# databricks/spark-deep-learning

Measured on AMD Instinct MI355X. Metric: images/sec, higher is better.
Workload: dtype bf16; 1 GPU; model=resnet50, global_batch=512, image=224, parallelism=dp1

## Files before the change

sparkdl/models/resnet.py:

```python

import torch
import torch.nn as nn

from sparkdl.ops import BatchNormAct2d, Conv1x1, batch_norm_relu_maxpool


class Bottleneck(nn.Module):
    expansion = 4

    def __init__(self, cin, width, stride=1):
        super().__init__()
        cout = width * self.expansion
        self.conv1 = Conv1x1(cin, width)
        self.bn1 = BatchNormAct2d(width, relu=True)
        self.conv2 = nn.Conv2d(width, width, 3, stride=stride, padding=1,
                               bias=False)
        self.bn2 = BatchNormAct2d(width, relu=True)
        self.conv3 = Conv1x1(width, cout)
        self.bn3 = BatchNormAct2d(cout, relu=True)
        if stride != 1 or cin != cout:
            self.down_conv = Conv1x1(cin, cout, stride=stride)
            self.down_bn = BatchNormAct2d(cout, relu=False)
        else:
            self.down_conv = None

    def forward(self, x):
        if self.down_conv is not None:
            idn = self.down_bn(self.down_conv(x))
        else:
            idn = x
        out = self.bn1(self.conv1(x))
        out = self.bn2(self.conv2(out))
        return self.bn3(self.conv3(out), residual=idn)


class ResNet50(nn.Module):
    LAYERS = (3, 4, 6, 3)

    def __init__(self, num_classes=1000):
        super().__init__()
        self.stem_conv = nn.Conv2d(3, 64, 7, stride=2, padding=3,
                                   bias=False)
        self.stem_bn = BatchNormAct2d(64, relu=True)
        self.stem_pool = nn.MaxPool2d(3, stride=2, padding=1)
        cin = 64
        stages = []
        for i, blocks in enumerate(self.LAYERS):
            width = 64 * (2 ** i)
            stride = 1 if i == 0 else 2
            layer = []
            for b in range(blocks):
                layer.append(Bottleneck(cin, width, stride if b == 0 else 1))
                cin = width * Bottleneck.expansion
            stages.append(nn.Sequential(*layer))
        self.stages = nn.Sequential(*stages)
        self.pool = nn.AdaptiveAvgPool2d(1)
        self.fc = nn.Linear(2048, num_classes)

        for m in self.modules():
            if isinstance(m, nn.Conv2d):
                nn.init.kaiming_normal_(m.weight, mode="fan_out",
                                        nonlinearity="relu")
        for m in self.modules():
            if isinstance(m, Bottleneck):
                nn.init.zeros_(m.bn3.weight)

    def forward(self, x):
        bn = self.stem_bn
        x = batch_norm_relu_maxpool(
            self.stem_conv(x), bn.weight, bn.bias, bn.running_mean,
            bn.running_var, momentum=bn.momentum, eps=bn.eps,
            training=bn.training)
        x = self.stages(x)
        x = self.pool(x).flatten(1)
        return self.fc(x)
```

sparkdl/ops/csrc/batchnorm.hip:

```cpp

#include "common.hip.h"
#include "kernels.h"

namespace {

constexpr int kBlock = 256;
constexpr int kVec = 8;
constexpr int kUnroll = 2;
constexpr int kFoldFloats = kBlock * 2 * kVec;
constexpr int kFinCh = 4;

__device__ __forceinline__ float bn_affine(short x, float scale,
                                           float shift) {
  return bf2f(x) * scale + shift;
}
__device__ __forceinline__ float bn_xhat(short x, float mean, float rstd) {
  return (bf2f(x) - mean) * rstd;
}
__device__ __forceinline__ float bn_dx(float d, float xh, float k1,
                                       float k2, float k3) {
  return k1 * (d - k2 - xh * k3);
}


// ... 247 lines not shown
      if (RELU) mbits = mask[base / kVec];
      accum(xv, dv, mbits);
    }
  }
  bn_block_fold(lds, s1, s2, rpb, row_off, lane_col, cols,
                slab + (size_t)blockIdx.x * 2 * cols);
}

__global__ __launch_bounds__(kBlock) void bn_bwd_finalize_k(
    const float* __restrict__ slab, int G, const float* __restrict__ gamma,
    const float* __restrict__ save_rstd, float* __restrict__ dgamma,
    float* __restrict__ dbeta, float* __restrict__ c1,
    float* __restrict__ c2, float* __restrict__ c3, long long rows,
    int cols, int training) {
  __shared__ float red[kBlock / WAVE * 2 * kFinCh];
  float sum_dym, sum_dymxh;
  const int blk = bn_fin_block();
  bn_slab_sum(slab, G, cols, blk, red, sum_dym, sum_dymxh);
  if (threadIdx.x >= kFinCh) return;
  const int c = blk * kFinCh + threadIdx.x;
  dgamma[c] = sum_dymxh;
  dbeta[c] = sum_dym;
  c1[c] = gamma[c] * save_rstd[c];
  if (training) {
    c2[c] = sum_dym / rows;
    c3[c] = sum_dymxh / rows;
  } else {
    c2[c] = 0.f;
    c3[c] = 0.f;
  }
}

template <bool RELU, bool RES>
__global__ __launch_bounds__(kBlock) void bn_bwd_apply_k(
    const short* __restrict__ x, const unsigned char* __restrict__ mask,
    const short* __restrict__ dy, const float* __restrict__ save_mean,
    const float* __restrict__ save_rstd, const float* __restrict__ c1,
    const float* __restrict__ c2, const float* __restrict__ c3,
    short* __restrict__ dx, short* __restrict__ dres, long long rows,
    int cols) {
  const int tpr = cols / kVec;
  const int rpb = kBlock / min(tpr, kBlock);
  const int lane_col = (threadIdx.x % tpr) * kVec;
  const int row_off = threadIdx.x / tpr;
  if (row_off >= rpb) return;
  const float4v m0 = *(const float4v*)(save_mean + lane_col);
  const float4v m1 = *(const float4v*)(save_mean + lane_col + 4);
  const float4v r0 = *(const float4v*)(save_rstd + lane_col);
  const float4v r1 = *(const float4v*)(save_rstd + lane_col + 4);
  const float4v a0 = *(const float4v*)(c1 + lane_col);
  const float4v a1 = *(const float4v*)(c1 + lane_col + 4);
  const float4v b0 = *(const float4v*)(c2 + lane_col);
  const float4v b1 = *(const float4v*)(c2 + lane_col + 4);
  const float4v g0 = *(const float4v*)(c3 + lane_col);
  const float4v g1 = *(const float4v*)(c3 + lane_col + 4);

  for (long long r = (long long)blockIdx.x * rpb + row_off; r < rows;
       r += (long long)gridDim.x * rpb) {
    const long long base = r * cols + lane_col;
    const short8 xv = *(const short8*)(x + base);
    const short8 dv = *(const short8*)(dy + base);
    unsigned char mbits = 0xffu;
    if (RELU) mbits = mask[base / kVec];
    short8 odx, odr;
#pragma unroll
    for (int j = 0; j < kVec; ++j) {
      float d = bf2f(dv[j]);
      if (RELU && !(mbits & (1u << j))) d = 0.f;
      const float mean = j < 4 ? m0[j] : m1[j - 4];
      const float rstd = j < 4 ? r0[j] : r1[j - 4];
      const float xh = bn_xhat(xv[j], mean, rstd);
      const float k1 = j < 4 ? a0[j] : a1[j - 4];
      const float k2 = j < 4 ? b0[j] : b1[j - 4];
      const float k3 = j < 4 ? g0[j] : g1[j - 4];
      odx[j] = f2bf(bn_dx(d, xh, k1, k2, k3));
      if (RES) odr[j] = f2bf(d);
    }
    *(short8*)(dx + base) = odx;
    if (RES) *(short8*)(dres + base) = odr;
  }
}


typedef unsigned uint2v __attribute__((ext_vector_type(2)));

constexpr unsigned kPoolDead = 9;
constexpr unsigned kPoolNone = 0xffu;

struct PoolGeom {
  int H, W, Ho, Wo;
};

__global__ __launch_bounds__(kBlock) void bn_apply_pool_k(
    const short* __restrict__ x, const float* __restrict__ scale,
    const float* __restrict__ shift, short* __restrict__ pooled,
    unsigned char* __restrict__ code, long long orows, int cols,
    PoolGeom g) {
  const int tpr = cols / kVec;
  const int rpb = kBlock / min(tpr, kBlock);
  const int lane_col = (threadIdx.x % tpr) * kVec;
  const int row_off = threadIdx.x / tpr;
  if (row_off >= rpb) return;
  const float4v sc0 = *(const float4v*)(scale + lane_col);
  const float4v sc1 = *(const float4v*)(scale + lane_col + 4);
  const float4v sh0 = *(const float4v*)(shift + lane_col);
  const float4v sh1 = *(const float4v*)(shift + lane_col + 4);
  const unsigned opix = (unsigned)(g.Ho * g.Wo);

  for (long long o = (long long)blockIdx.x * rpb + row_off; o < orows;
       o += (long long)gridDim.x * rpb) {
    const unsigned n = (unsigned)o / opix;
    const unsigned rem = (unsigned)o - n * opix;
    const int oh = (int)(rem / (unsigned)g.Wo);
    const int ow = (int)(rem - (unsigned)oh * (unsigned)g.Wo);
    short8 v[9];
#pragma unroll
    for (int kh = 0; kh < 3; ++kh) {
      const int ih = min(max(2 * oh - 1 + kh, 0), g.H - 1);
#pragma unroll
      for (int kw = 0; kw < 3; ++kw) {
        const int iw = min(max(2 * ow - 1 + kw, 0), g.W - 1);
        const long long r = ((long long)n * g.H + ih) * g.W + iw;
        v[kh * 3 + kw] = *(const short8*)(x + r * cols + lane_col);
      }
    }
    float best[kVec], bestf[kVec];
    unsigned tap[kVec];
#pragma unroll
    for (int j = 0; j < kVec; ++j) {
      best[j] = -INFINITY;
      bestf[j] = 0.f;
      tap[j] = 0;
    }
#pragma unroll
    for (int kh = 0; kh < 3; ++kh) {
      const int ih = 2 * oh - 1 + kh;
      const bool hin = ih >= 0 && ih < g.H;
#pragma unroll
      for (int kw = 0; kw < 3; ++kw) {
        const int iw = 2 * ow - 1 + kw;
        const bool in = hin && iw >= 0 && iw < g.W;
#pragma unroll
        for (int j = 0; j < kVec; ++j) {
          const float f =
              bn_affine(v[kh * 3 + kw][j], j < 4 ? sc0[j] : sc1[j - 4],
                        j < 4 ? sh0[j] : sh1[j - 4]);
          const float q = bf2f(f2bf(fmaxf(f, 0.f)));
          if (in && q > best[j]) {
            best[j] = q;
            bestf[j] = f;
            tap[j] = kh * 3 + kw;
          }
        }
      }
    }
    short8 ov;
    unsigned c0 = 0, c1 = 0;
#pragma unroll
    for (int j = 0; j < kVec; ++j) {
      union { float f; unsigned u; } b;
      b.f = best[j];
      ov[j] = (short)(b.u >> 16);
      const unsigned c = bestf[j] > 0.f ? tap[j] : kPoolDead;
      if (j < 4) c0 |= c << (8 * j);
      else c1 |= c << (8 * (j - 4));
    }
// ... 147 lines not shown
      const float rstd = j < 4 ? r0[j] : r1[j - 4];
      const float xh = bn_xhat(xv[j], mean, rstd);
      const float k1 = j < 4 ? a0[j] : a1[j - 4];
      const float k2 = j < 4 ? b0[j] : b1[j - 4];
      const float k3 = j < 4 ? g0[j] : g1[j - 4];
      odx[j] = f2bf(bn_dx(d[j], xh, k1, k2, k3));
    }
    *(short8*)(dx + base) = odx;
  }
}

int bn_grid(long long rows, int cols) {
  const int tpr = cols / kVec;
  const int rpb = kBlock / min(tpr, kBlock);
  long long blocks = (rows + rpb - 1) / rpb;
  return (int)min(blocks, 2048LL);
}

}

int bn_reduce_blocks(long long rows, int cols) {
  const int tpr = cols / kVec;
  const int rpb = kBlock / min(tpr, kBlock);
  const long long row_blocks = (rows + rpb - 1) / rpb;
  const long long g = max(256LL, min(512LL, rows / 64));
  return (int)max(1LL, min(row_blocks, g));
}

long long bn_scratch_floats(long long rows, int cols) {
  return (long long)bn_reduce_blocks(rows, cols) * 2 * cols + 3LL * cols;
}

void launch_bn_fwd(const short* x, const short* res, const float* gamma,
                   const float* beta, float* running_mean,
                   float* running_var, float* save_mean, float* save_rstd,
                   float* scratch, short* y, unsigned char* mask,
                   long long rows, int cols, float momentum, float eps,
                   bool training, bool relu, hipStream_t stream) {
  const int grid = bn_grid(rows, cols);
  const int G = bn_reduce_blocks(rows, cols);
  if (training)
    hipLaunchKernelGGL(bn_stats_k<kUnroll>, dim3(G), dim3(kBlock), 0,
                       stream, x, scratch, rows, cols);
  float* scale = scratch + (size_t)G * 2 * cols;
  float* shift = scale + cols;
  hipLaunchKernelGGL(bn_finalize_k, dim3(cols / kFinCh), dim3(kBlock), 0,
                     stream, scratch, G, gamma, beta, running_mean,
                     running_var, save_mean, save_rstd, scale, shift, rows,
                     cols, momentum, eps, (int)training);
  auto ap = relu ? (res ? bn_apply_k<true, true> : bn_apply_k<true, false>)
                 : (res ? bn_apply_k<false, true>
                        : bn_apply_k<false, false>);
  hipLaunchKernelGGL(ap, dim3(grid), dim3(kBlock), 0, stream, x, res,
                     scale, shift, y, mask, rows, cols);
}

void launch_bn_bwd(const short* x, const unsigned char* mask,
                   const short* dy, const float* gamma,
                   const float* save_mean, const float* save_rstd,
                   float* scratch, float* dgamma, float* dbeta, short* dx,
                   short* dres, long long rows, int cols, bool training,
                   bool relu, hipStream_t stream) {
  const int grid = bn_grid(rows, cols);
  const int G = bn_reduce_blocks(rows, cols);
  auto rk = relu ? bn_bwd_reduce_k<true, kUnroll>
                 : bn_bwd_reduce_k<false, kUnroll>;
  hipLaunchKernelGGL(rk, dim3(G), dim3(kBlock), 0, stream, x, mask, dy,
                     save_mean, save_rstd, scratch, rows, cols);
  float* c1 = scratch + (size_t)G * 2 * cols;
  float* c2 = c1 + cols;
  float* c3 = c2 + cols;
  hipLaunchKernelGGL(bn_bwd_finalize_k, dim3(cols / kFinCh), dim3(kBlock),
                     0, stream, scratch, G, gamma, save_rstd, dgamma, dbeta,
                     c1, c2, c3, rows, cols, (int)training);
  auto ak = relu ? (dres ? bn_bwd_apply_k<true, true>
                         : bn_bwd_apply_k<true, false>)
                 : (dres ? bn_bwd_apply_k<false, true>
                         : bn_bwd_apply_k<false, false>);
  hipLaunchKernelGGL(ak, dim3(grid), dim3(kBlock), 0, stream, x, mask, dy,
                     save_mean, save_rstd, c1, c2, c3, dx, dres, rows,
                     cols);
}

void launch_bn_pool_fwd(const short* x, const float* gamma,
                        const float* beta, float* running_mean,
                        float* running_var, float* save_mean,
                        float* save_rstd, float* scratch, short* pooled,
                        unsigned char* code, int n, int h, int w, int cols,
                        float momentum, float eps, bool training,
                        hipStream_t stream) {
  const PoolGeom g{h, w, (h - 1) / 2 + 1, (w - 1) / 2 + 1};
  const long long rows = (long long)n * h * w;
  const long long orows = (long long)n * g.Ho * g.Wo;
  const int G = bn_reduce_blocks(rows, cols);
  if (training)
    hipLaunchKernelGGL(bn_stats_k<kUnroll>, dim3(G), dim3(kBlock), 0,
                       stream, x, scratch, rows, cols);
  float* scale = scratch + (size_t)G * 2 * cols;
  float* shift = scale + cols;
  hipLaunchKernelGGL(bn_finalize_k, dim3(cols / kFinCh), dim3(kBlock), 0,
                     stream, scratch, G, gamma, beta, running_mean,
                     running_var, save_mean, save_rstd, scale, shift, rows,
                     cols, momentum, eps, (int)training);
  hipLaunchKernelGGL(bn_apply_pool_k, dim3(bn_grid(orows, cols)),
                     dim3(kBlock), 0, stream, x, scale, shift, pooled, code,
                     orows, cols, g);
}

void launch_bn_pool_bwd(const short* x, const unsigned char* code,
                        const short* dyp, const float* gamma,
                        const float* save_mean, const float* save_rstd,
                        float* scratch, float* dgamma, float* dbeta,
                        short* dx, int n, int h, int w, int cols,
                        bool training, hipStream_t stream) {
  const PoolGeom g{h, w, (h - 1) / 2 + 1, (w - 1) / 2 + 1};
  const long long rows = (long long)n * h * w;
  const int G = bn_reduce_blocks(rows, cols);
  hipLaunchKernelGGL(bn_pool_bwd_reduce_k<kUnroll>, dim3(G), dim3(kBlock),
                     0, stream, x, code, dyp, save_mean, save_rstd, scratch,
                     rows, cols, g);
  float* c1 = scratch + (size_t)G * 2 * cols;
  float* c2 = c1 + cols;
  float* c3 = c2 + cols;
  hipLaunchKernelGGL(bn_bwd_finalize_k, dim3(cols / kFinCh), dim3(kBlock),
                     0, stream, scratch, G, gamma, save_rstd, dgamma, dbeta,
                     c1, c2, c3, rows, cols, (int)training);
  hipLaunchKernelGGL(bn_pool_bwd_apply_k, dim3(bn_grid(rows, cols)),
                     dim3(kBlock), 0, stream, x, code, dyp, save_mean,
                     save_rstd, c1, c2, c3, dx, rows, cols, g);
}
```

sparkdl/ops/csrc/bindings.cpp:

```cpp

#include <torch/extension.h>
#include <ATen/hip/impl/HIPStreamMasqueradingAsCUDA.h>
#include <ATen/hip/impl/HIPGuardImplMasqueradingAsCUDA.h>

#include <cmath>
#include <vector>

#include "kernels.h"

namespace {

using DeviceGuard = c10::hip::HIPGuardMasqueradingAsCUDA;

hipStream_t cur_stream() {
  return c10::hip::getCurrentHIPStreamMasqueradingAsCUDA().stream();
}

#define CHECK_BF16_CUDA(t)                                            \
  TORCH_CHECK((t).is_cuda(), #t " must be on GPU");                   \
  TORCH_CHECK((t).scalar_type() == at::kBFloat16, #t " must be bf16");\
  TORCH_CHECK((t).is_contiguous(), #t " must be contiguous")

#define CHECK_F32_CUDA(t)                                             \
  TORCH_CHECK((t).is_cuda(), #t " must be on GPU");                   \
// ... 104 lines not shown
      cur_stream());
  return {dx, dgamma, dbeta};
}


std::vector<at::Tensor> bn_fwd(const at::Tensor& x,
                               const c10::optional<at::Tensor>& res,
                               const at::Tensor& gamma,
                               const at::Tensor& beta,
                               at::Tensor running_mean,
                               at::Tensor running_var, double momentum,
                               double eps, bool training, bool relu) {
  CHECK_BF16_CUDA(x);
  CHECK_F32_CUDA(gamma);
  CHECK_F32_CUDA(beta);
  DeviceGuard guard(x.device());
  const int cols = (int)x.size(-1);
  const long long rows = x.numel() / cols;
  TORCH_CHECK(cols % 8 == 0 && cols <= 2048,
              "bn_fwd requires cols%8==0 and cols<=2048 (NHWC channels)");
  const short* res_ptr = nullptr;
  if (res.has_value()) {
    CHECK_BF16_CUDA(res.value());
    TORCH_CHECK(res->sizes() == x.sizes());
    res_ptr = bf_ptr(res.value());
  }
  auto f32 = x.options().dtype(at::kFloat);
  auto y = at::empty_like(x);
  auto save_mean = at::empty({cols}, f32);
  auto save_rstd = at::empty({cols}, f32);
  auto scratch = at::empty({bn_scratch_floats(rows, cols)}, f32);
  at::Tensor mask;
  unsigned char* mask_ptr = nullptr;
  if (relu) {
    mask = at::empty({rows * cols / 8}, x.options().dtype(at::kByte));
    mask_ptr = mask.data_ptr<unsigned char>();
  } else {
    mask = at::empty({0}, x.options().dtype(at::kByte));
  }
  launch_bn_fwd(bf_ptr(x), res_ptr, gamma.data_ptr<float>(),
                beta.data_ptr<float>(), running_mean.data_ptr<float>(),
                running_var.data_ptr<float>(), save_mean.data_ptr<float>(),
                save_rstd.data_ptr<float>(), scratch.data_ptr<float>(),
                bf_ptr_mut(y), mask_ptr, rows, cols, (float)momentum,
                (float)eps, training, relu, cur_stream());
  return {y, save_mean, save_rstd, mask};
}

std::vector<at::Tensor> bn_bwd(const at::Tensor& x,
                               const at::Tensor& mask,
                               const at::Tensor& dy,
                               const at::Tensor& gamma,
                               const at::Tensor& save_mean,
                               const at::Tensor& save_rstd, bool training,
                               bool relu, bool needs_dres) {
  CHECK_BF16_CUDA(x);
  CHECK_BF16_CUDA(dy);
  CHECK_F32_CUDA(gamma);
  DeviceGuard guard(x.device());
  const int cols = (int)x.size(-1);
  const long long rows = x.numel() / cols;
  TORCH_CHECK(!relu || mask.numel() == rows * cols / 8,
              "relu backward needs the forward's activation mask");
  auto f32 = x.options().dtype(at::kFloat);
  auto dx = at::empty_like(x);
  auto dgamma = at::empty({cols}, f32);
  auto dbeta = at::empty({cols}, f32);
  auto scratch = at::empty({bn_scratch_floats(rows, cols)}, f32);
  at::Tensor dres;
  short* dres_ptr = nullptr;
  if (needs_dres) {
    dres = at::empty_like(x);
    dres_ptr = bf_ptr_mut(dres);
  }
  launch_bn_bwd(bf_ptr(x),
                relu ? mask.data_ptr<unsigned char>() : nullptr,
                bf_ptr(dy), gamma.data_ptr<float>(),
                save_mean.data_ptr<float>(), save_rstd.data_ptr<float>(),
                scratch.data_ptr<float>(), dgamma.data_ptr<float>(),
                dbeta.data_ptr<float>(), bf_ptr_mut(dx), dres_ptr, rows,
                cols, training, relu, cur_stream());
  if (needs_dres) return {dx, dgamma, dbeta, dres};
  return {dx, dgamma, dbeta};
}

std::vector<at::Tensor> bn_pool_fwd(const at::Tensor& x,
                                    const at::Tensor& gamma,
                                    const at::Tensor& beta,
                                    at::Tensor running_mean,
                                    at::Tensor running_var, double momentum,
                                    double eps, bool training) {
  CHECK_BF16_CUDA(x);
  CHECK_F32_CUDA(gamma);
  CHECK_F32_CUDA(beta);
  CHECK_F32_CUDA(running_mean);
  CHECK_F32_CUDA(running_var);
  TORCH_CHECK(x.dim() == 4, "bn_pool_fwd takes x as [N,H,W,C]");
  DeviceGuard guard(x.device());
  const int64_t n = x.size(0), h = x.size(1), w = x.size(2);
  const int cols = (int)x.size(3);
  TORCH_CHECK(cols % 8 == 0 && cols <= 2048,
              "bn_pool_fwd requires cols%8==0 and cols<=2048");
  TORCH_CHECK(n > 0 && h > 0 && w > 0 && n * h * w < (1LL << 31),
              "bn_pool_fwd requires 0 < N*H*W < 2^31");
  TORCH_CHECK(gamma.numel() == cols && beta.numel() == cols &&
              running_mean.numel() == cols && running_var.numel() == cols);
  const int64_t ho = (h - 1) / 2 + 1, wo = (w - 1) / 2 + 1;
  auto f32 = x.options().dtype(at::kFloat);
  auto pooled = at::empty({n, ho, wo, cols}, x.options());
  auto code = at::empty({n, ho, wo, cols}, x.options().dtype(at::kByte));
  auto save_mean = at::empty({cols}, f32);
  auto save_rstd = at::empty({cols}, f32);
  auto scratch = at::empty({bn_scratch_floats(n * h * w, cols)}, f32);
  launch_bn_pool_fwd(bf_ptr(x), gamma.data_ptr<float>(),
                     beta.data_ptr<float>(), running_mean.data_ptr<float>(),
                     running_var.data_ptr<float>(),
                     save_mean.data_ptr<float>(),
                     save_rstd.data_ptr<float>(), scratch.data_ptr<float>(),
                     bf_ptr_mut(pooled), code.data_ptr<unsigned char>(),
                     (int)n, (int)h, (int)w, cols, (float)momentum,
                     (float)eps, training, cur_stream());
  return {pooled, save_mean, save_rstd, code};
}

std::vector<at::Tensor> bn_pool_bwd(const at::Tensor& x,
                                    const at::Tensor& code,
                                    const at::Tensor& dyp,
                                    const at::Tensor& gamma,
                                    const at::Tensor& save_mean,
                                    const at::Tensor& save_rstd,
                                    bool training) {
  CHECK_BF16_CUDA(x);
  CHECK_BF16_CUDA(dyp);
  CHECK_F32_CUDA(gamma);
  CHECK_F32_CUDA(save_mean);
  CHECK_F32_CUDA(save_rstd);
  TORCH_CHECK(x.dim() == 4, "bn_pool_bwd takes x as [N,H,W,C]");
  DeviceGuard guard(x.device());
  const int64_t n = x.size(0), h = x.size(1), w = x.size(2);
  const int cols = (int)x.size(3);
  TORCH_CHECK(cols % 8 == 0 && cols <= 2048,
              "bn_pool_bwd requires cols%8==0 and cols<=2048");
  TORCH_CHECK(n > 0 && h > 0 && w > 0 && n * h * w < (1LL << 31),
              "bn_pool_bwd requires 0 < N*H*W < 2^31");
  const int64_t ho = (h - 1) / 2 + 1, wo = (w - 1) / 2 + 1;
  const std::vector<int64_t> pshape = {n, ho, wo, (int64_t)cols};
  TORCH_CHECK(dyp.sizes() == at::IntArrayRef(pshape),
              "pooled grad must be [N,Ho,Wo,C]");
  TORCH_CHECK(code.is_cuda() && code.scalar_type() == at::kByte &&
              code.is_contiguous() &&
              code.sizes() == at::IntArrayRef(pshape),
              "backward needs the forward's tap codes");
  TORCH_CHECK(gamma.numel() == cols && save_mean.numel() == cols &&
              save_rstd.numel() == cols);
  auto f32 = x.options().dtype(at::kFloat);
  auto dx = at::empty_like(x);
  auto dgamma = at::empty({cols}, f32);
  auto dbeta = at::empty({cols}, f32);
  auto scratch = at::empty({bn_scratch_floats(n * h * w, cols)}, f32);
  launch_bn_pool_bwd(bf_ptr(x), code.data_ptr<unsigned char>(),
                     bf_ptr(dyp), gamma.data_ptr<float>(),
                     save_mean.data_ptr<float>(),
                     save_rstd.data_ptr<float>(), scratch.data_ptr<float>(),
                     dgamma.data_ptr<float>(), dbeta.data_ptr<float>(),
                     bf_ptr_mut(dx), (int)n, (int)h, (int)w, cols, training,
                     cur_stream());
// ... 244 lines not shown
}

at::Tensor wgrad_splitk(const at::Tensor& dZ, const at::Tensor& X) {
  CHECK_BF16_CUDA(dZ);
  CHECK_BF16_CUDA(X);
  TORCH_CHECK(dZ.dim() == 2 && X.dim() == 2 && dZ.size(0) == X.size(0));
  const long long M = dZ.size(0);
  const int N = (int)dZ.size(1), K = (int)X.size(1);
  TORCH_CHECK(wgrad_splitk_supported(M, N, K),
              "wgrad_splitk requires N%256==0, K%128==0, M%64==0");
  DeviceGuard guard(dZ.device());
  auto dW = at::empty({N, K}, dZ.options().dtype(at::kFloat));
  launch_wgrad_splitk(bf_ptr(dZ), bf_ptr(X), dW.data_ptr<float>(), M, N,
                      K, cur_stream());
  return dW;
}

at::Tensor transpose_bf16(const at::Tensor& X) {
  CHECK_BF16_CUDA(X);
  TORCH_CHECK(X.dim() == 2 && X.is_contiguous());
  DeviceGuard guard(X.device());
  const int R = (int)X.size(0), C = (int)X.size(1);
  auto Y = at::empty({C, R}, X.options());
  launch_transpose_bf16(bf_ptr(X), bf_ptr_mut(Y), R, C, cur_stream());
  return Y;
}


at::Tensor gbt_histogram(const at::Tensor& B, const at::Tensor& g,
                         const at::Tensor& h, const at::Tensor& row_list,
                         const at::Tensor& bmap, int64_t n_nodes) {
  TORCH_CHECK(B.is_cuda() && B.scalar_type() == at::kByte &&
              B.is_contiguous());
  CHECK_F32_CUDA(g);
  CHECK_F32_CUDA(h);
  TORCH_CHECK(row_list.is_cuda() && row_list.scalar_type() == at::kInt);
  TORCH_CHECK(bmap.is_cuda() && bmap.scalar_type() == at::kInt &&
              bmap.size(-1) == 4);
  DeviceGuard guard(B.device());
  const int F = (int)B.size(1);
  TORCH_CHECK(F % 8 == 0, "feature dim must be padded to a multiple of 8");
  auto hist = at::zeros({n_nodes, F, 256, 2},
                        B.options().dtype(at::kFloat));
  launch_gbt_histogram(
      B.data_ptr<unsigned char>(), g.data_ptr<float>(),
      h.data_ptr<float>(), row_list.data_ptr<int>(),
      reinterpret_cast<const int4*>(bmap.data_ptr<int>()),
      (int)(bmap.numel() / 4), F, hist.data_ptr<float>(), cur_stream());
  return hist;
}

}

PYBIND11_MODULE(TORCH_EXTENSION_NAME, m) {
  m.doc() = "sparkdl MI355X-native kernels (gfx950)";
  m.def("fused_adamw_", &fused_adamw_, "Fused multi-tensor AdamW step");
  m.def("fused_sgd_", &fused_sgd_, "Fused multi-tensor SGD step");
  m.def("zero_grads_", &zero_grads_, "Zero all grads in a chunk table");
  m.def("gemm_bias_act", &gemm_bias_act, "MFMA GEMM + bias(+GELU) (N6)");
  m.def("transpose_bf16", &transpose_bf16, "bf16 2D transpose (dgrad W^T)");
  m.def("gemm_stream", &gemm_stream,
        "Streaming tall-skinny GEMM (1x1 convs)");
  m.def("wgrad_splitk", &wgrad_splitk,
        "Split-M wgrad GEMM (tr_b16 fragment path)");
  m.def("attn_fwd", &attn_fwd, "Flash attention fwd (D=64, bf16)",
        py::arg("q"), py::arg("k"), py::arg("v"), py::arg("dropout_p"),
        py::arg("seed"), py::arg("seqlens") = py::none());
  m.def("attn_bwd", &attn_bwd, "Flash attention bwd (dQ/dK/dV)",
        py::arg("q"), py::arg("k"), py::arg("v"), py::arg("dO"),
        py::arg("lse"), py::arg("drow"), py::arg("dropout_p"),
        py::arg("seed"), py::arg("seqlens") = py::none());
  m.def("attn_fwd_packed", &attn_fwd_packed,
        "Flash attention fwd over the packed qkv buffer", py::arg("qkv"),
        py::arg("dropout_p"), py::arg("seed"),
        py::arg("seqlens") = py::none());
  m.def("attn_bwd_packed", &attn_bwd_packed,
        "Flash attention bwd -> packed dqkv", py::arg("qkv"),
        py::arg("dO"), py::arg("lse"), py::arg("drow"),
        py::arg("dropout_p"), py::arg("seed"),
        py::arg("seqlens") = py::none());
  m.def("gbt_histogram", &gbt_histogram, "GBT g/h histogram (N7)");
  m.def("bn_fwd", &bn_fwd, "Fused BatchNorm(+add)(+ReLU) fwd (bf16 NHWC)");
  m.def("bn_bwd", &bn_bwd, "Fused BatchNorm(+add)(+ReLU) bwd (bf16 NHWC)");
  m.def("bn_pool_fwd", &bn_pool_fwd,
        "Fused BatchNorm+ReLU+MaxPool(3,2,1) fwd (bf16 NHWC)");
  m.def("bn_pool_bwd", &bn_pool_bwd,
        "Fused BatchNorm+ReLU+MaxPool(3,2,1) bwd (bf16 NHWC)");
  m.def("layernorm_fwd", &layernorm_fwd, "LayerNorm forward (bf16)");
  m.def("layernorm_bwd", &layernorm_bwd, "LayerNorm backward (bf16)");
  m.def("bias_gelu_fwd", &bias_gelu_fwd, "Fused bias+GELU forward (bf16)");
  m.def("bias_gelu_bwd", &bias_gelu_bwd, "Fused bias+GELU backward (bf16)");
  m.attr("_chunk_elems") = kOptChunk;
}
```

sparkdl/ops/csrc/kernels.h:

```cpp
#pragma once

#include <hip/hip_runtime.h>
#include <cstdint>

struct TensorChunk {
  float* p;
  const float* g;
  float* m;
  float* v;
  long long n;
  short* pl;
};

constexpr int kOptChunk = 16384;

void launch_fused_adamw(const TensorChunk* chunks, const int2* bmap,
                        int nblocks, float lr, float beta1, float beta2,
                        float eps, float weight_decay,
                        long long* step_counter, float* coeffs,
                        hipStream_t stream);

void launch_fused_sgd(const TensorChunk* chunks, const int2* bmap,
                      int nblocks, float lr, float momentum,
                      float weight_decay, bool nesterov, bool first_step,
                      hipStream_t stream);

void launch_layernorm_fwd(const short* x, const float* gamma,
                          const float* beta, short* y, float* save_mean,
                          float* save_rstd, int rows, int cols, float eps,
                          hipStream_t stream);

void launch_layernorm_bwd(const short* x, const short* dy,
                          const float* gamma, const float* save_mean,
                          const float* save_rstd, short* dx,
                          float* dgamma_part, float* dbeta_part,
                          int part_rows, int rows, int cols,
                          hipStream_t stream);

int layernorm_bwd_part_rows(int rows);

void launch_layernorm_reduce_parts(const float* dgamma_part,
                                   const float* dbeta_part, float* dgamma,
                                   float* dbeta, int part_rows, int cols,
                                   hipStream_t stream);

void launch_bias_gelu_fwd(const short* x, const float* bias, short* y,
                          long long rows, int cols, hipStream_t stream);

void launch_bias_gelu_bwd(const short* x, const float* bias,
                          const short* dy, short* dx, float* dbias,
                          long long rows, int cols, hipStream_t stream);

int bn_reduce_blocks(long long rows, int cols);
long long bn_scratch_floats(long long rows, int cols);

void launch_bn_fwd(const short* x, const short* res, const float* gamma,
                   const float* beta, float* running_mean,
                   float* running_var, float* save_mean, float* save_rstd,
                   float* scratch, short* y, unsigned char* mask,
                   long long rows, int cols, float momentum, float eps,
                   bool training, bool relu, hipStream_t stream);

void launch_bn_bwd(const short* x, const unsigned char* mask,
                   const short* dy, const float* gamma,
                   const float* save_mean, const float* save_rstd,
                   float* scratch, float* dgamma, float* dbeta, short* dx,
                   short* dres, long long rows, int cols, bool training,
                   bool relu, hipStream_t stream);

void launch_bn_pool_fwd(const short* x, const float* gamma,
                        const float* beta, float* running_mean,
                        float* running_var, float* save_mean,
                        float* save_rstd, float* scratch, short* pooled,
                        unsigned char* code, int n, int h, int w, int cols,
                        float momentum, float eps, bool training,
                        hipStream_t stream);

void launch_bn_pool_bwd(const short* x, const unsigned char* code,
                        const short* dyp, const float* gamma,
                        const float* save_mean, const float* save_rstd,
                        float* scratch, float* dgamma, float* dbeta,
                        short* dx, int n, int h, int w, int cols,
                        bool training, hipStream_t stream);

void launch_gemm_bias_act(const short* A, const short* W,
                          const float* bias, short* C, short* Z, int M,
                          int N, int K, int act, hipStream_t stream);
bool gemm_bias_act_supported(int M, int N, int K);

void launch_gemm_stream(const short* A, const short* W, short* C,
                        long long M, int N, int K, hipStream_t stream);
bool gemm_stream_supported(long long M, int N, int K);

void launch_wgrad_splitk(const short* dZ, const short* X, float* dW,
                         long long M, int N, int K, hipStream_t stream);
bool wgrad_splitk_supported(long long M, int N, int K);

void launch_transpose_bf16(const short* X, short* Y, int R, int C,
                           hipStream_t stream);

void launch_attn_pretranspose(const short* X, short* T, int BH, int S,
                              int H, int rs, hipStream_t stream);
void launch_attn_fwd(const short* Q, const short* K, const short* VT,
                     short* O, float* LSE, const long long* seed, int BH,
                     int S, int H, int rs, int ors, float dropout_p,
                     const int* seqlens, hipStream_t stream);
void launch_attn_bwd(const short* Q, const short* K, const short* V,
                     const short* dO, const short* QT, const short* DOT,
                     const short* KT, const float* LSE, const float* Drow,
                     short* dQ, short* dK, short* dV,
                     const long long* seed, int BH, int S, int H, int rs,
                     int ors, int grs, float dropout_p,
                     const int* seqlens, hipStream_t stream);

void launch_gbt_histogram(const unsigned char* B, const float* g,
                          const float* h, const int* row_list,
                          const int4* bmap, int nblocks, int F,
                          float* hist, hipStream_t stream);

void launch_zero_grads(const TensorChunk* chunks, const int2* bmap,
                       int nblocks, hipStream_t stream);
```

sparkdl/ops/functional.py:

```python

import os

import torch

import sparkdl.ops as _ops



def layer_norm_ref(x, gamma, beta, eps=1e-5):
    xf = x.float()
    out = torch.nn.functional.layer_norm(
        xf, (x.shape[-1],), gamma.float(), beta.float(), eps)
    return out.to(x.dtype)


def bias_gelu_ref(x, bias):
    return torch.nn.functional.gelu(
        x.float() + bias.float(), approximate="none").to(x.dtype)


def masked_attention_ref(q, k, v, seq_lens, dropout_p=0.0):
    S, d = q.shape[-2], q.shape[-1]
    qf, kf, vf = q.float(), k.float(), v.float()
    lens = torch.as_tensor(seq_lens, device=q.device).clamp(0, S)
    lens = lens.reshape((-1,) + (1,) * (q.dim() - 2))
    valid = torch.arange(S, device=q.device) < lens
    kmask = valid.unsqueeze(-2)
    qmask = valid.unsqueeze(-1)
    with torch.autocast(q.device.type, enabled=False):
        s = qf @ kf.transpose(-1, -2) / d ** 0.5
        s = s.masked_fill(~kmask, torch.finfo(torch.float32).min)
        p = torch.softmax(s, dim=-1)
        p = torch.where(kmask & qmask, p, p.new_zeros(()))
        if dropout_p > 0:
            p = torch.nn.functional.dropout(p, dropout_p)
        o = p @ vf
    return o.to(q.dtype)


def seqlens_from_mask(attention_mask, validate=None):
    m = attention_mask
    if m.dim() != 2:
        raise ValueError("attention_mask must be [B, S], got %s"
                         % (tuple(m.shape),))
    mb = m != 0
    lens = mb.sum(-1, dtype=torch.int32)
    if validate is None:
        validate = not (m.is_cuda
                        and torch.cuda.is_current_stream_capturing())
    if validate:
        prefix = torch.arange(m.shape[1], device=m.device) \
            < lens.unsqueeze(-1)
        if not bool((mb == prefix).all()):
            raise ValueError(
                "attention_mask must be right-padded: every row a run "
                "of ones followed by zeros (no holes, no left padding)")
    return lens



class _LayerNormFn(torch.autograd.Function):
    @staticmethod
    def forward(ctx, x, gamma, beta, eps):
        C = _ops.ext()
        x = x.contiguous()
        y, mean, rstd = C.layernorm_fwd(x, gamma, beta, eps)
        ctx.save_for_backward(x, gamma, mean, rstd)
        return y

    @staticmethod
    def backward(ctx, dy):
        C = _ops.ext()
        x, gamma, mean, rstd = ctx.saved_tensors
        dx, dgamma, dbeta = C.layernorm_bwd(
            x, dy.contiguous(), gamma, mean, rstd)
        return dx, dgamma, dbeta, None


class _BiasGeluFn(torch.autograd.Function):
    @staticmethod
    def forward(ctx, x, bias):
        C = _ops.ext()
        x = x.contiguous()
        ctx.save_for_backward(x, bias)
        return C.bias_gelu_fwd(x, bias)

    @staticmethod
    def backward(ctx, dy):
        C = _ops.ext()
        x, bias = ctx.saved_tensors
        dx, dbias = C.bias_gelu_bwd(x, bias, dy.contiguous())
        return dx, dbias


def _to_nhwc(t):
    return t.permute(0, 2, 3, 1).contiguous(memory_format=torch.contiguous_format)


def _from_nhwc(t):
    return t.permute(0, 3, 1, 2)


class _BNReLUFn(torch.autograd.Function):
    @staticmethod
    def forward(ctx, x, residual, gamma, beta, running_mean, running_var,
                momentum, eps, training, relu):
        C = _ops.ext()
        xp = _to_nhwc(x)
        rp = _to_nhwc(residual) if residual is not None else None
        y, mean, rstd, mask = C.bn_fwd(
            xp, rp, gamma, beta, running_mean, running_var, momentum,
            eps, training, relu)
        ctx.save_for_backward(xp, mask, gamma, mean, rstd)
        ctx.bn_flags = (training, relu, residual is not None)
        return _from_nhwc(y)

    @staticmethod
    def backward(ctx, dy):
        C = _ops.ext()
        xp, mask, gamma, mean, rstd = ctx.saved_tensors
        training, relu, has_res = ctx.bn_flags
        needs_dres = has_res and ctx.needs_input_grad[1]
        outs = C.bn_bwd(xp, mask, _to_nhwc(dy), gamma, mean, rstd,
                        training, relu, needs_dres)
        dx = _from_nhwc(outs[0])
        dres = _from_nhwc(outs[3]) if needs_dres else None
        return (dx, dres, outs[1], outs[2], None, None, None, None, None,
                None)


def batch_norm_act(x, gamma, beta, running_mean, running_var,
                   momentum=0.1, eps=1e-5, training=True, relu=False,
                   residual=None):
    C = x.shape[1]
    if (x.is_cuda and x.dtype == torch.bfloat16
            and C <= 2048 and C % 8 == 0):
        return _BNReLUFn.apply(x, residual, gamma, beta, running_mean,
                               running_var, momentum, eps, training, relu)
    y = torch.nn.functional.batch_norm(
        x.float(), running_mean, running_var, gamma, beta,
        training, momentum, eps).to(x.dtype)
    if residual is not None:
        y = y + residual
    return torch.relu(y) if relu else y


class _BNReLUPoolFn(torch.autograd.Function):

    @staticmethod
    def forward(ctx, x, gamma, beta, running_mean, running_var, momentum,
                eps, training):
        C = _ops.ext()
        xp = _to_nhwc(x)
        pooled, mean, rstd, code = C.bn_pool_fwd(
            xp, gamma, beta, running_mean, running_var, momentum, eps,
            training)
        ctx.save_for_backward(xp, code, gamma, mean, rstd)
        ctx.bn_training = training
        return _from_nhwc(pooled)

    @staticmethod
    def backward(ctx, dy):
        C = _ops.ext()
        xp, code, gamma, mean, rstd = ctx.saved_tensors
        dx, dgamma, dbeta = C.bn_pool_bwd(
            xp, code, _to_nhwc(dy), gamma, mean, rstd, ctx.bn_training)
        return _from_nhwc(dx), dgamma, dbeta, None, None, None, None, None


def batch_norm_relu_maxpool(x, gamma, beta, running_mean, running_var,
                            momentum=0.1, eps=1e-5, training=True):
    C = x.shape[1]
    if (x.is_cuda and x.dtype == torch.bfloat16 and x.dim() == 4
            and C <= 2048 and C % 8 == 0
            and 0 < x.numel() // C < 2 ** 31
            and os.environ.get("SPARKDL_FUSED_STEM", "1") != "0"):
        return _BNReLUPoolFn.apply(x, gamma, beta, running_mean,
                                   running_var, momentum, eps, training)
    y = batch_norm_act(x, gamma, beta, running_mean, running_var,
                       momentum=momentum, eps=eps, training=training,
                       relu=True)
    return torch.nn.functional.max_pool2d(y, 3, stride=2, padding=1)


def layer_norm(x, gamma, beta, eps=1e-5):
    if x.is_cuda and x.dtype == torch.bfloat16:
        return _LayerNormFn.apply(x, gamma, beta, eps)
    return torch.nn.functional.layer_norm(
        x, (x.shape[-1],), gamma.to(x.dtype), beta.to(x.dtype), eps)


def bias_gelu(x, bias):
    if x.is_cuda and x.dtype == torch.bfloat16:
        return _BiasGeluFn.apply(x, bias)
    return torch.nn.functional.gelu(x + bias.to(x.dtype), approximate="none")



_zero_bias_cache = {}


def _zero_bias(n, device):
    key = (n, device)
    if key not in _zero_bias_cache:
        _zero_bias_cache[key] = torch.zeros(
            n, dtype=torch.float32, device=device)
    return _zero_bias_cache[key]


class _LinearGeluFusedFn(torch.autograd.Function):

    @staticmethod
    def forward(ctx, x2d, weight, bias):
        C = _ops.ext()
        y, z = C.gemm_bias_act(x2d, weight, bias, 1, True)
        ctx.save_for_backward(x2d, weight, z)
        return y

    @staticmethod
    def backward(ctx, dy):
        C = _ops.ext()
        x2d, weight, z = ctx.saved_tensors
        dy = dy.contiguous()
        dz, dbias = C.bias_gelu_bwd(z, _zero_bias(z.shape[-1], z.device),
                                    dy)
        if (weight.shape[0] % 64 == 0
                and os.environ.get("SPARKDL_FUSED_DGRAD", "1") != "0"):
# ... 211 lines not shown
```

sparkdl/ops/modules.py:

```python

import torch
import torch.nn as nn

from sparkdl.ops import functional as F_


class LayerNorm(nn.Module):
    def __init__(self, hidden, eps=1e-5):
        super().__init__()
        self.weight = nn.Parameter(torch.ones(hidden, dtype=torch.float32))
        self.bias = nn.Parameter(torch.zeros(hidden, dtype=torch.float32))
        self.eps = eps

    def forward(self, x):
        return F_.layer_norm(x, self.weight, self.bias, self.eps)

    def extra_repr(self):
        return "%d, eps=%g" % (self.weight.numel(), self.eps)


class BatchNormAct2d(nn.Module):

    def __init__(self, num_features, eps=1e-5, momentum=0.1, relu=False):
        super().__init__()
        self.num_features = num_features
        self.eps = eps
        self.momentum = momentum
        self.relu = relu
        self.weight = nn.Parameter(
            torch.ones(num_features, dtype=torch.float32))
        self.bias = nn.Parameter(
            torch.zeros(num_features, dtype=torch.float32))
        self.register_buffer(
            "running_mean", torch.zeros(num_features, dtype=torch.float32))
        self.register_buffer(
            "running_var", torch.ones(num_features, dtype=torch.float32))

    def forward(self, x, residual=None):
        return F_.batch_norm_act(
            x, self.weight, self.bias, self.running_mean, self.running_var,
            momentum=self.momentum, eps=self.eps, training=self.training,
            relu=self.relu, residual=residual)

    def extra_repr(self):
        return "%d, relu=%s" % (self.num_features, self.relu)


def convert_bf16_training(model):
    for mod in model.modules():
        if isinstance(mod, (nn.Linear, nn.Embedding)):
            mod.to(torch.bfloat16)
        elif isinstance(mod, (Linear, LinearGelu)):
            mod.weight.data = mod.weight.data.bfloat16()
    return model


class LinearGelu(nn.Module):

    def __init__(self, in_features, out_features):
        super().__init__()
        self.weight = nn.Parameter(torch.empty(out_features, in_features))
        self.bias = nn.Parameter(torch.zeros(out_features, dtype=torch.float32))
        nn.init.normal_(self.weight, std=0.02)

    def forward(self, x):
        import os
        if (os.environ.get("SPARKDL_FUSED_GEMM", "1") != "0"
                and F_.linear_gelu_fused_ok(x, self.weight)):
            return F_.linear_gelu_fused(x, self.weight, self.bias)
        h = torch.nn.functional.linear(x, self.weight.to(x.dtype))
        return F_.bias_gelu(h, self.bias)


class Linear(nn.Module):

    def __init__(self, in_features, out_features, bias=True):
        super().__init__()
        self.in_features = in_features
        self.out_features = out_features
        self.weight = nn.Parameter(torch.empty(out_features, in_features))
        self.bias = nn.Parameter(
            torch.zeros(out_features, dtype=torch.float32)) if bias \
            else None
        nn.init.normal_(self.weight, std=0.02)

    def forward(self, x):
        import os
        if (os.environ.get("SPARKDL_FUSED_GEMM", "1") != "0"
                and F_.linear_gelu_fused_ok(x, self.weight)):
            return F_.linear_fused(x, self.weight, self.bias)
        y = torch.nn.functional.linear(x, self.weight.to(x.dtype))
        if self.bias is not None:
            y = y + self.bias.to(y.dtype)
        return y

    def extra_repr(self):
        return "%d, %d, bias=%s" % (self.in_features, self.out_features,
                                    self.bias is not None)


class Conv1x1(nn.Module):

    def __init__(self, cin, cout, stride=1):
        super().__init__()
        self.cin, self.cout, self.stride = cin, cout, stride
        self.weight = nn.Parameter(torch.empty(cout, cin))
        nn.init.kaiming_normal_(self.weight, mode="fan_out",
                                nonlinearity="relu")

    def forward(self, x):
        import os
        mode = os.environ.get("SPARKDL_CONV1X1", "0")
        use = (self.stride == 1 and x.is_cuda
               and x.dtype == torch.bfloat16 and self.cin % 64 == 0
               and mode != "0"
               and (mode == "all" or self.cin >= 512))
        if use:
            xp = x.permute(0, 2, 3, 1)
            y = F_.conv1x1_gemm(xp, self.weight.to(x.dtype))
            return y.permute(0, 3, 1, 2)
        w4 = self.weight.view(self.cout, self.cin, 1, 1)
        return torch.nn.functional.conv2d(x, w4.to(x.dtype),
                                          stride=self.stride)

    def extra_repr(self):
# ... 2 lines not shown
```

Baseline: 9713 images/s.

## Fuse residual-branch gradient sum into BatchNorm backward via forked outputs

Each bottleneck's final BN returns two aliased outputs, one for the main path and one for the skip path. Autograd therefore hands both gradients straight to the BN backward instead of summing them with a separate add. A new bn_bwd2 path sums the two gradients inside the reduce kernel, stores the sum for reuse as the residual gradient, and applies the BN backward from it. This removes an elementwise add pass per block. It adds aliasing tricks with set_ and set_materialize_grads(False), and it rounds the summed gradient to bf16 before the statistics.

```diff
diff --git a/sparkdl/models/resnet.py b/sparkdl/models/resnet.py
--- a/sparkdl/models/resnet.py
+++ b/sparkdl/models/resnet.py
@@ -25,13 +25,14 @@
             self.down_conv = None
 
     def forward(self, x):
+        x, skip = x if isinstance(x, tuple) else (x, x)
         if self.down_conv is not None:
-            idn = self.down_bn(self.down_conv(x))
+            idn = self.down_bn(self.down_conv(skip))
         else:
-            idn = x
+            idn = skip
         out = self.bn1(self.conv1(x))
         out = self.bn2(self.conv2(out))
-        return self.bn3(self.conv3(out), residual=idn)
+        return self.bn3(self.conv3(out), residual=idn, fork=True)
 
 
 class ResNet50(nn.Module):
@@ -71,6 +72,6 @@
             self.stem_conv(x), bn.weight, bn.bias, bn.running_mean,
             bn.running_var, momentum=bn.momentum, eps=bn.eps,
             training=bn.training)
-        x = self.stages(x)
+        x, _ = self.stages(x)
         x = self.pool(x).flatten(1)
         return self.fc(x)
diff --git a/sparkdl/ops/csrc/batchnorm.hip b/sparkdl/ops/csrc/batchnorm.hip
--- a/sparkdl/ops/csrc/batchnorm.hip
+++ b/sparkdl/ops/csrc/batchnorm.hip
@@ -353,6 +353,118 @@
 }
 
 
+template <bool RELU, int U>
+__global__ __launch_bounds__(kBlock) void bn_bwd2_reduce_k(
+    const short* __restrict__ x, const unsigned char* __restrict__ mask,
+    const short* __restrict__ dya, const short* __restrict__ dyb,
+    const float* __restrict__ save_mean,
+    const float* __restrict__ save_rstd, short* __restrict__ s,
+    float* __restrict__ slab, long long rows, int cols) {
+  __shared__ __attribute__((aligned(16))) float lds[kFoldFloats];
+  const int tpr = cols / kVec;
+  const int rpb = kBlock / min(tpr, kBlock);
+  const int lane_col = (threadIdx.x % tpr) * kVec;
+  const int row_off = threadIdx.x / tpr;
+
+  float s1[kVec] = {0.f}, s2[kVec] = {0.f};
+  if (row_off < rpb) {
+    const float4v m0 = *(const float4v*)(save_mean + lane_col);
+    const float4v m1 = *(const float4v*)(save_mean + lane_col + 4);
+    const float4v r0 = *(const float4v*)(save_rstd + lane_col);
+    const float4v r1 = *(const float4v*)(save_rstd + lane_col + 4);
+    auto accum = [&](const short8& xv, const short8& ua, const short8& ub,
+                     unsigned char mbits, long long base) {
+      short8 sv;
+#pragma unroll
+      for (int j = 0; j < kVec; ++j) {
+        short sb = f2bf(bf2f(ua[j]) + bf2f(ub[j]));
+        if (RELU && !(mbits & (1u << j))) sb = 0;
+        sv[j] = sb;
+        const float d = bf2f(sb);
+        const float mean = j < 4 ? m0[j] : m1[j - 4];
+        const float rstd = j < 4 ? r0[j] : r1[j - 4];
+        const float xh = bn_xhat(xv[j], mean, rstd);
+        s1[j] += d;
+        s2[j] += d * xh;
+      }
+      *(short8*)(s + base) = sv;
+    };
+    const long long stride = (long long)gridDim.x * rpb;
+    long long r = (long long)blockIdx.x * rpb + row_off;
+    for (; r + (U - 1) * stride < rows; r += U * stride) {
+      short8 xv[U], ua[U], ub[U];
+      unsigned char mb[U];
+#pragma unroll
+      for (int u = 0; u < U; ++u) {
+        const long long base = (r + u * stride) * cols + lane_col;
+        xv[u] = *(const short8*)(x + base);
+        ua[u] = *(const short8*)(dya + base);
+        ub[u] = *(const short8*)(dyb + base);
+        mb[u] = 0xffu;
+        if (RELU) mb[u] = mask[base / kVec];
+      }
+#pragma unroll
+      for (int u = 0; u < U; ++u)
+        accum(xv[u], ua[u], ub[u], mb[u],
+              (r + u * stride) * cols + lane_col);
+    }
+    for (; r < rows; r += stride) {
+      const long long base = r * cols + lane_col;
+      const short8 xv = *(const short8*)(x + base);
+      const short8 ua = *(const short8*)(dya + base);
+      const short8 ub = *(const short8*)(dyb + base);
+      unsigned char mbits = 0xffu;
+      if (RELU) mbits = mask[base / kVec];
+      accum(xv, ua, ub, mbits, base);
+    }
+  }
+  bn_block_fold(lds, s1, s2, rpb, row_off, lane_col, cols,
+                slab + (size_t)blockIdx.x * 2 * cols);
+}
+
+__global__ __launch_bounds__(kBlock) void bn_bwd2_apply_k(
+    const short* __restrict__ x, const short* __restrict__ s,
+    const float* __restrict__ save_mean,
+    const float* __restrict__ save_rstd, const float* __restrict__ c1,
+    const float* __restrict__ c2, const float* __restrict__ c3,
+    short* __restrict__ dx, long long rows, int cols) {
+  const int tpr = cols / kVec;
+  const int rpb = kBlock / min(tpr, kBlock);
+  const int lane_col = (threadIdx.x % tpr) * kVec;
+  const int row_off = threadIdx.x / tpr;
+  if (row_off >= rpb) return;
+  const float4v m0 = *(const float4v*)(save_mean + lane_col);
+  const float4v m1 = *(const float4v*)(save_mean + lane_col + 4);
+  const float4v r0 = *(const float4v*)(save_rstd + lane_col);
+  const float4v r1 = *(const float4v*)(save_rstd + lane_col + 4);
+  const float4v a0 = *(const float4v*)(c1 + lane_col);
+  const float4v a1 = *(const float4v*)(c1 + lane_col + 4);
+  const float4v b0 = *(const float4v*)(c2 + lane_col);
+  const float4v b1 = *(const float4v*)(c2 + lane_col + 4);
+  const float4v g0 = *(const float4v*)(c3 + lane_col);
+  const float4v g1 = *(const float4v*)(c3 + lane_col + 4);
+
+  for (long long r = (long long)blockIdx.x * rpb + row_off; r < rows;
+       r += (long long)gridDim.x * rpb) {
+    const long long base = r * cols + lane_col;
+    const short8 xv = *(const short8*)(x + base);
+    const short8 sv = *(const short8*)(s + base);
+    short8 odx;
+#pragma unroll
+    for (int j = 0; j < kVec; ++j) {
+      const float mean = j < 4 ? m0[j] : m1[j - 4];
+      const float rstd = j < 4 ? r0[j] : r1[j - 4];
+      const float xh = bn_xhat(xv[j], mean, rstd);
+      const float k1 = j < 4 ? a0[j] : a1[j - 4];
+      const float k2 = j < 4 ? b0[j] : b1[j - 4];
+      const float k3 = j < 4 ? g0[j] : g1[j - 4];
+      odx[j] = f2bf(bn_dx(bf2f(sv[j]), xh, k1, k2, k3));
+    }
+    *(short8*)(dx + base) = odx;
+  }
+}
+
+
 typedef unsigned uint2v __attribute__((ext_vector_type(2)));
 
 constexpr unsigned kPoolDead = 9;
@@ -666,6 +778,29 @@
                      cols);
 }
 
+void launch_bn_bwd2(const short* x, const unsigned char* mask,
+                    const short* dya, const short* dyb, const float* gamma,
+                    const float* save_mean, const float* save_rstd,
+                    float* scratch, float* dgamma, float* dbeta, short* dx,
+                    short* s, long long rows, int cols, bool training,
+                    bool relu, hipStream_t stream) {
+  const int grid = bn_grid(rows, cols);
+  const int G = bn_reduce_blocks(rows, cols);
+  auto rk = relu ? bn_bwd2_reduce_k<true, kUnroll>
+                 : bn_bwd2_reduce_k<false, kUnroll>;
+  hipLaunchKernelGGL(rk, dim3(G), dim3(kBlock), 0, stream, x, mask, dya,
+                     dyb, save_mean, save_rstd, s, scratch, rows, cols);
+  float* c1 = scratch + (size_t)G * 2 * cols;
+  float* c2 = c1 + cols;
+  float* c3 = c2 + cols;
+  hipLaunchKernelGGL(bn_bwd_finalize_k, dim3(cols / kFinCh), dim3(kBlock),
+                     0, stream, scratch, G, gamma, save_rstd, dgamma, dbeta,
+                     c1, c2, c3, rows, cols, (int)training);
+  hipLaunchKernelGGL(bn_bwd2_apply_k, dim3(grid), dim3(kBlock), 0, stream,
+                     x, s, save_mean, save_rstd, c1, c2, c3, dx, rows,
+                     cols);
+}
+
 void launch_bn_pool_fwd(const short* x, const float* gamma,
                         const float* beta, float* running_mean,
                         float* running_var, float* save_mean,
diff --git a/sparkdl/ops/csrc/bindings.cpp b/sparkdl/ops/csrc/bindings.cpp
--- a/sparkdl/ops/csrc/bindings.cpp
+++ b/sparkdl/ops/csrc/bindings.cpp
@@ -210,6 +210,45 @@
                 cols, training, relu, cur_stream());
   if (needs_dres) return {dx, dgamma, dbeta, dres};
   return {dx, dgamma, dbeta};
+}
+
+std::vector<at::Tensor> bn_bwd2(const at::Tensor& x,
+                                const at::Tensor& mask,
+                                const at::Tensor& dy_a,
+                                const at::Tensor& dy_b,
+                                const at::Tensor& gamma,
+                                const at::Tensor& save_mean,
+                                const at::Tensor& save_rstd, bool training,
+                                bool relu) {
+  CHECK_BF16_CUDA(x);
+  CHECK_BF16_CUDA(dy_a);
+  CHECK_BF16_CUDA(dy_b);
+  CHECK_F32_CUDA(gamma);
+  TORCH_CHECK(dy_a.sizes() == x.sizes() && dy_b.sizes() == x.sizes(),
+              "bn_bwd2: both gradients must have x's shape");
+  DeviceGuard guard(x.device());
+  const int cols = (int)x.size(-1);
+  const long long rows = x.numel() / cols;
+  TORCH_CHECK(cols % 8 == 0 && cols <= 2048,
+              "bn_bwd2 requires cols%8==0 and cols<=2048 (NHWC channels)");
+  TORCH_CHECK(!relu || mask.numel() == rows * cols / 8,
+              "relu backward needs the forward's activation mask");
+  TORCH_CHECK(gamma.numel() == cols && save_mean.numel() == cols &&
+              save_rstd.numel() == cols);
+  auto f32 = x.options().dtype(at::kFloat);
+  auto dx = at::empty_like(x);
+  auto s = at::empty_like(x);
+  auto dgamma = at::empty({cols}, f32);
+  auto dbeta = at::empty({cols}, f32);
+  auto scratch = at::empty({bn_scratch_floats(rows, cols)}, f32);
+  launch_bn_bwd2(bf_ptr(x),
+                 relu ? mask.data_ptr<unsigned char>() : nullptr,
+                 bf_ptr(dy_a), bf_ptr(dy_b), gamma.data_ptr<float>(),
+                 save_mean.data_ptr<float>(), save_rstd.data_ptr<float>(),
+                 scratch.data_ptr<float>(), dgamma.data_ptr<float>(),
+                 dbeta.data_ptr<float>(), bf_ptr_mut(dx), bf_ptr_mut(s),
+                 rows, cols, training, relu, cur_stream());
+  return {dx, dgamma, dbeta, s};
 }
 
 std::vector<at::Tensor> bn_pool_fwd(const at::Tensor& x,
@@ -620,6 +659,8 @@
   m.def("gbt_histogram", &gbt_histogram, "GBT g/h histogram (N7)");
   m.def("bn_fwd", &bn_fwd, "Fused BatchNorm(+add)(+ReLU) fwd (bf16 NHWC)");
   m.def("bn_bwd", &bn_bwd, "Fused BatchNorm(+add)(+ReLU) bwd (bf16 NHWC)");
+  m.def("bn_bwd2", &bn_bwd2,
+        "Fused BatchNorm(+add)(+ReLU) bwd over the sum of two gradients");
   m.def("bn_pool_fwd", &bn_pool_fwd,
         "Fused BatchNorm+ReLU+MaxPool(3,2,1) fwd (bf16 NHWC)");
   m.def("bn_pool_bwd", &bn_pool_bwd,
diff --git a/sparkdl/ops/csrc/kernels.h b/sparkdl/ops/csrc/kernels.h
--- a/sparkdl/ops/csrc/kernels.h
+++ b/sparkdl/ops/csrc/kernels.h
@@ -68,6 +68,13 @@
                    short* dres, long long rows, int cols, bool training,
                    bool relu, hipStream_t stream);
 
+void launch_bn_bwd2(const short* x, const unsigned char* mask,
+                    const short* dya, const short* dyb, const float* gamma,
+                    const float* save_mean, const float* save_rstd,
+                    float* scratch, float* dgamma, float* dbeta, short* dx,
+                    short* s, long long rows, int cols, bool training,
+                    bool relu, hipStream_t stream);
+
 void launch_bn_pool_fwd(const short* x, const float* gamma,
                         const float* beta, float* running_mean,
                         float* running_var, float* save_mean,
diff --git a/sparkdl/ops/functional.py b/sparkdl/ops/functional.py
--- a/sparkdl/ops/functional.py
+++ b/sparkdl/ops/functional.py
@@ -101,10 +101,16 @@
     return t.permute(0, 3, 1, 2)
 
 
+def _alias(t):
+    return torch.empty(0, dtype=t.dtype, device=t.device).set_(
+        t.untyped_storage(), t.storage_offset(), t.size(), t.stride())
+
+
 class _BNReLUFn(torch.autograd.Function):
+
     @staticmethod
     def forward(ctx, x, residual, gamma, beta, running_mean, running_var,
-                momentum, eps, training, relu):
+                momentum, eps, training, relu, fork=False):
         C = _ops.ext()
         xp = _to_nhwc(x)
         rp = _to_nhwc(residual) if residual is not None else None
@@ -113,36 +119,55 @@
             eps, training, relu)
         ctx.save_for_backward(xp, mask, gamma, mean, rstd)
         ctx.bn_flags = (training, relu, residual is not None)
-        return _from_nhwc(y)
-
-    @staticmethod
-    def backward(ctx, dy):
+        out = _from_nhwc(y)
+        if not fork:
+            return out
+        ctx.set_materialize_grads(False)
+        return _alias(out), _alias(out)
+
+    @staticmethod
+    def backward(ctx, dy, dy2=None):
         C = _ops.ext()
         xp, mask, gamma, mean, rstd = ctx.saved_tensors
         training, relu, has_res = ctx.bn_flags
         needs_dres = has_res and ctx.needs_input_grad[1]
-        outs = C.bn_bwd(xp, mask, _to_nhwc(dy), gamma, mean, rstd,
-                        training, relu, needs_dres)
+        if dy is None:
+            dy, dy2 = dy2, None
+        if dy is None:
+            return (None,) * 11
+        if dy2 is not None:
+            outs = C.bn_bwd2(xp, mask, _to_nhwc(dy), _to_nhwc(dy2), gamma,
+                             mean, rstd, training, relu)
+        else:
+            outs = C.bn_bwd(xp, mask, _to_nhwc(dy), gamma, mean, rstd,
+                            training, relu, needs_dres)
         dx = _from_nhwc(outs[0])
         dres = _from_nhwc(outs[3]) if needs_dres else None
         return (dx, dres, outs[1], outs[2], None, None, None, None, None,
-                None)
+                None, None)
 
 
 def batch_norm_act(x, gamma, beta, running_mean, running_var,
                    momentum=0.1, eps=1e-5, training=True, relu=False,
-                   residual=None):
+                   residual=None, fork=False):
     C = x.shape[1]
     if (x.is_cuda and x.dtype == torch.bfloat16
             and C <= 2048 and C % 8 == 0):
-        return _BNReLUFn.apply(x, residual, gamma, beta, running_mean,
-                               running_var, momentum, eps, training, relu)
+        if fork and os.environ.get("SPARKDL_FUSED_RESGRAD", "1") != "0":
+            return _BNReLUFn.apply(x, residual, gamma, beta, running_mean,
+                                   running_var, momentum, eps, training,
+                                   relu, True)
+        y = _BNReLUFn.apply(x, residual, gamma, beta, running_mean,
+                            running_var, momentum, eps, training, relu,
+                            False)
+        return (y, y) if fork else y
     y = torch.nn.functional.batch_norm(
         x.float(), running_mean, running_var, gamma, beta,
         training, momentum, eps).to(x.dtype)
     if residual is not None:
         y = y + residual
-    return torch.relu(y) if relu else y
+    y = torch.relu(y) if relu else y
+    return (y, y) if fork else y
 
 
 class _BNReLUPoolFn(torch.autograd.Function):
diff --git a/sparkdl/ops/modules.py b/sparkdl/ops/modules.py
--- a/sparkdl/ops/modules.py
+++ b/sparkdl/ops/modules.py
@@ -36,11 +36,11 @@
         self.register_buffer(
             "running_var", torch.ones(num_features, dtype=torch.float32))
 
-    def forward(self, x, residual=None):
+    def forward(self, x, residual=None, fork=False):
         return F_.batch_norm_act(
             x, self.weight, self.bias, self.running_mean, self.running_var,
             momentum=self.momentum, eps=self.eps, training=self.training,
-            relu=self.relu, residual=residual)
+            relu=self.relu, residual=residual, fork=fork)
 
     def extra_repr(self):
         return "%d, relu=%s" % (self.num_features, self.relu)
```

After: 9951 images/s, median of 6. +2.4%, better.
